# maxwerhahn/Multi-pass-GAN

Measured on AMD Instinct MI355X. Metric: volumes/sec (4x two-pass generator inference, 64^3->256^3 density-only), higher is better.
Workload: dtype f16+2xbf6->f32

## Files before the change

multi-pass-gan_amd/csrc/mpgan_conv_f6.hip:

```cpp
#include "mpgan_conv.h"

using namespace mpg::conv;

namespace {

#ifndef MPG_AH
#define MPG_AH 2
#endif
#ifndef MPG_WD
#define MPG_WD 1
#endif
#ifndef MPG_DIAG6
#define MPG_DIAG6 0
#endif
#ifndef MPG_W0
#define MPG_W0 1
#endif
#ifndef MPG_IMG_LATE
#define MPG_IMG_LATE 0
#endif
#ifndef MPG_PIECES_AFTER
#define MPG_PIECES_AFTER 1
#endif
#ifndef MPG_ALT
#define MPG_ALT 0
#endif
#ifndef MPG_STAMPS
#define MPG_STAMPS 0
#endif
#if MPG_STAMPS
#define MPG_STAMP(v) asm volatile("s_memtime %0" : "=s"(v))
#else
#define MPG_STAMP(v)
#endif
constexpr int lo_step(int pt, int nt, int ptn) {
    const int s = nt - ptn + pt - 1;
    return s < 0 ? 0 : (s > nt - 1 ? nt - 1 : s);
}

typedef int v16i __attribute__((ext_vector_type(16)));
typedef int v8i __attribute__((ext_vector_type(8)));
typedef int v6i __attribute__((ext_vector_type(6)));
typedef _Float16 half32 __attribute__((ext_vector_type(32)));
typedef _Float16 half16 __attribute__((ext_vector_type(16)));

__device__ __forceinline__ v8i lds_read32(const char* p) {
    const v4i lo = *reinterpret_cast<const v4i*>(p);
    const v4i hi = *reinterpret_cast<const v4i*>(p + 1024);
    return __builtin_shufflevector(lo, hi, 0, 1, 2, 3, 4, 5, 6, 7);
}

template <int OFF, class T>
__device__ __forceinline__ void ds_read16(T& dst, unsigned addr) {
    static_assert(sizeof(T) == 16 && OFF >= 0 && OFF < 65536, "one ds_read_b128");
    asm volatile("ds_read_b128 %0, %1 offset:%2" : "=v"(dst) : "v"(addr), "n"(OFF));
}

constexpr int kx_cum(int h, int NT, int PT) { return h + PT * ((h + NT - 1) / NT); }
constexpr int kx_allowed(int g, int NT, int PT, int AH) {
    const int G16 = 4 * NT;
    const int hi = g + AH + 1 < G16 ? g + AH + 1 : G16;
    return kx_cum(hi, NT, PT) - kx_cum(g + 1, NT, PT);
}

__device__ __forceinline__ half32 cat32(const half8& a, const half8& b, const half8& c, const half8& d) {
    const half16 lo = __builtin_shufflevector(a, b, 0, 1, 2, 3, 4, 5, 6, 7, 8, 9, 10, 11, 12, 13, 14, 15);
    const half16 hi = __builtin_shufflevector(c, d, 0, 1, 2, 3, 4, 5, 6, 7, 8, 9, 10, 11, 12, 13, 14, 15);
    return __builtin_shufflevector(lo, hi, 0, 1, 2, 3, 4, 5, 6, 7, 8, 9, 10, 11, 12, 13, 14, 15, 16, 17, 18, 19, 20, 21, 22, 23,
                                   24, 25, 26, 27, 28, 29, 30, 31);
}

__device__ __forceinline__ int block_exp16(const half32& v) {
    const v16i r = __builtin_bit_cast(v16i, v);
    int a0, a1, a2, a3, a4, a5, a6, a7, b0, b1, b2, b3, b4, b5, b6, b7, m2, m1;
#define MPG_MAX3(d, x, y, z) asm("v_pk_maximum3_f16 %0, %1, %2, %3" : "=v"(d) : "v"(x), "v"(y), "v"(z))
#define MPG_MIN3(d, x, y, z) asm("v_pk_minimum3_f16 %0, %1, %2, %3" : "=v"(d) : "v"(x), "v"(y), "v"(z))
    MPG_MAX3(a0, r[0], r[1], r[2]); MPG_MAX3(a1, r[3], r[4], r[5]); MPG_MAX3(a2, r[6], r[7], r[8]); MPG_MAX3(a3, r[9], r[10], r[11]);
    MPG_MAX3(a4, r[12], r[13], r[14]); MPG_MAX3(a5, a0, a1, r[15]); MPG_MAX3(a6, a2, a3, a4); MPG_MAX3(a7, a5, a6, a6);
    MPG_MIN3(b0, r[0], r[1], r[2]); MPG_MIN3(b1, r[3], r[4], r[5]); MPG_MIN3(b2, r[6], r[7], r[8]); MPG_MIN3(b3, r[9], r[10], r[11]);
    MPG_MIN3(b4, r[12], r[13], r[14]); MPG_MIN3(b5, b0, b1, r[15]); MPG_MIN3(b6, b2, b3, b4); MPG_MIN3(b7, b5, b6, b6);
#undef MPG_MAX3
#undef MPG_MIN3
    asm("v_pk_max_f16 %0, %1, %2 neg_lo:[0,1] neg_hi:[0,1]" : "=v"(m2) : "v"(a7), "v"(b7));
    asm("v_pk_max_f16 %0, %1, %1 op_sel:[0,1] op_sel_hi:[1,0]" : "=v"(m1) : "v"(m2));
    return (m1 >> 10) & 31;
}

#ifndef MPG_CVT_DIVIDES
#define MPG_CVT_DIVIDES 1
#endif
__device__ __forceinline__ float pow2_from_byte(int e8m0) {
#if MPG_CVT_DIVIDES
    return __builtin_bit_cast(float, e8m0 << 23);
#else
    return __builtin_bit_cast(float, (254 - e8m0) << 23);
#endif
}
__device__ __forceinline__ v8i widen6(const v6i& v) {
    return __builtin_shufflevector(v, v, 0, 1, 2, 3, 4, 5, -1, -1);
}
__device__ __forceinline__ v8i bf6_of(const half32& v, int e8m0) {
    return widen6(__builtin_amdgcn_cvt_scalef32_pk32_bf6_f16(v, pow2_from_byte(e8m0)));
}
constexpr int BF6 = 3;

template <int NT>
__global__ __launch_bounds__(Pipe6<NT>::WAVES * 64, Pipe6<NT>::OCC) void conv_mfma_f6_kernel(const ConvArgs a_unused) {
    extern __shared__ __attribute__((aligned(16))) char smem[];
    const KArgs ap = (KArgs)__builtin_amdgcn_kernarg_segment_ptr();
    const auto& a = *ap;
    using P = Pipe6<NT>;
    constexpr int WAVES = P::WAVES, PT = P::PT, TH = P::TH, WF16 = P::WF16, WF6 = P::WF6, WSTAGE = P::WSTAGE;
    constexpr int NI = P::NI, R = P::R, D = P::D, THREADS = WAVES * 64;
    constexpr bool FLAT = NT == 1;

    int* tap16 = reinterpret_cast<int*>(smem);
    char* img_lds = smem + a.tap_bytes;
    char* w_lds = img_lds + 2 * a.img_bytes;

    const int tid = threadIdx.x;
    const int lane = tid & 63;
    const int wave = tid >> 6;
    const int wave_u = __builtin_amdgcn_readfirstlane(wave);
    const int r = lane & 31;
    const int hh = lane >> 5;

    int bid = blockIdx.x;
    const int nblk = gridDim.x;
    if ((nblk & 7) == 0) bid = (bid & 7) * (nblk >> 3) + (bid >> 3);
    const int tx = bid % a.tiles_x;
    const int t2 = bid / a.tiles_x;
    const int ty = t2 % a.tiles_y;
    const int n = t2 / a.tiles_y;
    const int y0 = ty * TH, x0 = tx * TW;

    f32x16 acc[PT][NT];
#pragma unroll
    for (int pt = 0; pt < PT; ++pt)
#pragma unroll
        for (int nt = 0; nt < NT; ++nt)
#pragma unroll
            for (int i = 0; i < 16; ++i) acc[pt][nt][i] = 0.f;

    const EpiPre pre = epilogue_prefetch(ap, tid);
    const int seg_flip = (NT == 1 && a.nseg > 1) ? ((int)(blockIdx.x >> 8) & 1) : 0;
    for (int s0 = 0; s0 < ((a.dbg & 1) ? 0 : a.nseg); ++s0) {
        const int s = seg_flip ? a.nseg - 1 - s0 : s0;
        const auto& sg = ap->seg[s];
        if (NT <= 2 && sg.direct) {
            const unsigned plane_bytes = (unsigned)(sg.hs * sg.ws) * 16u;
            const unsigned gstride = 2u * plane_bytes;
            const char* xb = sg.x + ((size_t)n * sg.cg_total + sg.g_off) * gstride;
            unsigned pixo[PT];
#pragma unroll
            for (int pt = 0; pt < PT; ++pt) {
                int yy = y0 + PT * wave + pt, xx = x0 + r;
                yy = (yy < a.h ? yy : a.h - 1) >> sg.upy;
                xx = (xx < a.w ? xx : a.w - 1) >> sg.up;
                pixo[pt] = (unsigned)(yy * sg.ws + xx) * 16u;
            }
            const int glast = sg.cg_seg - 1;
            auto dma_stage_d = [&](int stage) {
                const int sidx = stage < sg.sc ? stage : sg.sc - 1;
                const char* src = sg.w + (size_t)sidx * WSTAGE + tid * 16;
                char* dst = w_lds + (stage % R) * WSTAGE + wave_u * 1024;
#pragma unroll
                for (int i = 0; i < NI; ++i) dma16(src + i * (THREADS * 16), dst + i * (THREADS * 16));
            };
#pragma unroll
            for (int d = 0; d < D; ++d) dma_stage_d(d);
            for (int st = 0; st < sg.sc; ++st) {
                wait_dma_and_barrier<(D - 1) * NI>();
                dma_stage_d(st + D);
                const char* wb = w_lds + (st % R) * WSTAGE;
                const char* xs = xb + (size_t)st * 8 * gstride;
                const int grem = glast - st * 8;
                if constexpr (FLAT) {
                    const unsigned a_base = lds_off(wb) + (unsigned)lane * 16u;
                    const char* xs_hi = xs;
                    const char* xs_lo = xs + plane_bytes;
                    asm volatile("" : "+s"(xs_hi), "+s"(xs_lo));
                    static_for<0, PT>([&](auto qc) {
                        constexpr int q = decltype(qc)::value;
                        half8 b_hi[4], b_lo[4], aq[2];
                        v4i wl[2], wh[2];
#pragma unroll
                        for (int j = 0; j < 4; ++j) {
                            int g = 2 * j + hh;
                            g = g < grem ? g : grem;
                            const unsigned vo = pixo[q] + g * gstride;
                            typedef const __attribute__((address_space(1))) half8* gmem;
                            b_hi[j] = __builtin_nontemporal_load((gmem)(xs_hi + vo));
                            b_lo[j] = __builtin_nontemporal_load((gmem)(xs_lo + vo));
                        }
                        ds_read16<0>(aq[0], a_base);
                        ds_read16<1024>(aq[1], a_base);
                        static_for<0, 4>([&](auto jc) {
                            constexpr int j = decltype(jc)::value;
                            lgkm_wait<(j < 3 ? 1 : 2)>();
                            tie(aq[j & 1]);
                            acc[q][0] = __builtin_amdgcn_mfma_f32_32x32x16_f16(aq[j & 1], b_hi[j], acc[q][0], 0, 0, 0);
                            if constexpr (j < 2) {
                                ds_read16<(j + 2) * 1024>(aq[j & 1], a_base);
                            } else if constexpr (j == 2) {
                                ds_read16<WF16 + WF6>(wl[0], a_base);
                                ds_read16<WF16 + WF6 + 1024>(wl[1], a_base);
                            } else {
                                ds_read16<WF16>(wh[0], a_base);
                                ds_read16<WF16 + 1024>(wh[1], a_base);
                            }
                        });
                        const half32 bh = cat32(b_hi[0], b_hi[1], b_hi[2], b_hi[3]);
                        const int e = block_exp16(bh);
                        const v8i hi6 = bf6_of(bh, e + 109);
                        const v8i lo6 = bf6_of(cat32(b_lo[0], b_lo[1], b_lo[2], b_lo[3]), e + 97);
                        const int sb = (e + 109) | (e + 97) << 8;
                        lgkm_wait<2>();
                        tie(wl[0]);
                        tie(wl[1]);
                        const v8i w_lo = __builtin_shufflevector(wl[0], wl[1], 0, 1, 2, 3, 4, 5, 6, 7);
                        acc[q][0] = __builtin_amdgcn_mfma_scale_f32_32x32x64_f8f6f4(w_lo, hi6, acc[q][0], BF6, BF6, 1, w_lo[6], 0, sb);
                        lgkm_wait<0>();
                        tie(wh[0]);
                        tie(wh[1]);
                        const v8i w_hi = __builtin_shufflevector(wh[0], wh[1], 0, 1, 2, 3, 4, 5, 6, 7);
                        acc[q][0] = __builtin_amdgcn_mfma_scale_f32_32x32x64_f8f6f4(w_hi, lo6, acc[q][0], BF6, BF6, 0, w_hi[6], 1, sb);
                    });
                    continue;
                }
                constexpr int PH = 2;
                static_for<0, PT / PH>([&](auto hc) {
                    constexpr int p0 = decltype(hc)::value * PH;
                    half8 b_hi[4][PH], b_lo[4][PH];
#pragma unroll
                    for (int j = 0; j < 4; ++j) {
                        int g = 2 * j + hh;
                        g = g < grem ? g : grem;
#pragma unroll
                        for (int q = 0; q < PH; ++q) {
                            b_hi[j][q] = __builtin_nontemporal_load(reinterpret_cast<const half8*>(xs + (pixo[p0 + q] + g * gstride)));
                            b_lo[j][q] = __builtin_nontemporal_load(reinterpret_cast<const half8*>(xs + (pixo[p0 + q] + g * gstride + plane_bytes)));
                        }
                    }
#pragma unroll
                    for (int j = 0; j < 4; ++j) {
#pragma unroll
                        for (int nt = 0; nt < NT; ++nt) {
                            const half8 a_hi = *reinterpret_cast<const half8*>(wb + ((j * NT + nt) * 64 + lane) * 16);
#pragma unroll
                            for (int q = 0; q < PH; ++q)
                                acc[p0 + q][nt] = __builtin_amdgcn_mfma_f32_32x32x16_f16(a_hi, b_hi[j][q], acc[p0 + q][nt], 0, 0, 0);
                        }
                    }
                    v8i hi6[PH], lo6[PH];
                    int sb[PH];
#pragma unroll
                    for (int q = 0; q < PH; ++q) {
                        const half32 bh = cat32(b_hi[0][q], b_hi[1][q], b_hi[2][q], b_hi[3][q]);
                        const half32 bl = cat32(b_lo[0][q], b_lo[1][q], b_lo[2][q], b_lo[3][q]);
                        const int e = block_exp16(bh);
                        hi6[q] = bf6_of(bh, e + 109);
                        lo6[q] = bf6_of(bl, e + 97);
                        sb[q] = (e + 109) | (e + 97) << 8;
                    }
#pragma unroll
                    for (int nt = 0; nt < NT; ++nt) {
                        const v8i w_hi = lds_read32(wb + WF16 + nt * 2048 + lane * 16);
                        const v8i w_lo = lds_read32(wb + WF16 + WF6 + nt * 2048 + lane * 16);
#pragma unroll
                        for (int q = 0; q < PH; ++q) {
                            acc[p0 + q][nt] = __builtin_amdgcn_mfma_scale_f32_32x32x64_f8f6f4(w_lo, hi6[q], acc[p0 + q][nt], BF6, BF6, 1, w_lo[6], 0, sb[q]);
                            acc[p0 + q][nt] = __builtin_amdgcn_mfma_scale_f32_32x32x64_f8f6f4(w_hi, lo6[q], acc[p0 + q][nt], BF6, BF6, 0, w_hi[6], 1, sb[q]);
                        }
                    }
                });
            }
            asm volatile("s_waitcnt vmcnt(0)" ::: "memory");
            __syncthreads();
            if constexpr (!FLAT) continue;
        }
        if constexpr (FLAT) {
            if (__builtin_amdgcn_readfirstlane(sg.direct)) continue;
        }
        const int T = sg.kh * sg.kw;
        const int G = sg.nchunks;
        const int NS = sg.sc;
        const int plane_b = sg.np * 16;
        const int ppg = sg.np >> 6;

        for (int q = tid; q < NS * 8; q += THREADS) {
            const int g = q / sg.tp;
            const int t = q - g * sg.tp;
            int off = ((g < G ? g : G - 1) & 1) * a.img_bytes;
            if (g < G && t < T) {
                const int dy = t / sg.kw;
                const int dx = t - dy * sg.kw;
                off += (dy * sg.iw + dx) * 16;
            }
            tap16[(q >> 3) * 8 + (q & 1) * 4 + ((q & 7) >> 1)] = off;
        }
        int pixb[PT];
#pragma unroll
        for (int pt = 0; pt < PT; ++pt) pixb[pt] = ((PT * wave + pt) * sg.iw + r) * 16;

        const size_t plane_px = (size_t)sg.hs * sg.ws;
        constexpr int MAXI = 4;
        static_assert(WAVES == 8, "MAXI");
        int img_src[MAXI];
#pragma unroll
        for (int i = 0; i < MAXI; ++i) {
            const int pc = WAVES * i + wave_u;
            const int pl = pc / ppg;
            const int p = (pc - pl * ppg) * 64 + lane;
            const int hy = p / sg.iw;
            const int hx = p - hy * sg.iw;
            const int yy = y0 - sg.pt + hy;
            const int xx = x0 - sg.pl + hx;
            const bool ok = pl < 2 && hy < sg.ih && yy >= 0 && yy < a.h && xx >= 0 && xx < a.w;
            img_src[i] = ok ? (int)(((size_t)pl * plane_px + (size_t)(yy >> sg.upy) * sg.ws + (xx >> sg.up)) * 16) : -1;
        }
        const size_t group_bytes = 2 * plane_px * 16;
        const char* const x_first = sg.x + ((size_t)n * sg.cg_total + sg.g_off) * group_bytes;
        auto img_piece = [&](int chunk, auto ic) {
            constexpr int i = decltype(ic)::value;
            if ((MPG_DIAG6 & 4) && chunk > 0) return;
            if (i < sg.ni_img) {
                const int off = img_src[i];
                const char* src = (off >= 0 && chunk < sg.cg_seg) ? x_first + (size_t)chunk * group_bytes + off : a.zeros;
                dma16_stream(src, img_lds + (chunk & 1) * a.img_bytes + (WAVES * i + wave_u) * 1024);
            }
        };
        auto w_piece = [&](int stage, auto ic) {
            constexpr int i = decltype(ic)::value;
            const int sidx = stage < NS ? stage : NS - 1;
            if ((MPG_DIAG6 & 8) && stage >= D) return;
            dma16(sg.w + (size_t)sidx * WSTAGE + tid * 16 + i * (THREADS * 16),
                  w_lds + (stage % R) * WSTAGE + wave_u * 1024 + i * (THREADS * 16));
        };
        static_for<0, MAXI>([&](auto ic) { img_piece(0, ic); });
#pragma unroll
        for (int d = 0; d < D; ++d) static_for<0, NI>([&](auto ic) { w_piece(d, ic); });
        int g_next = 1;

        half8 bh[PT][4];
        v4i o16n = {0, 0, 0, 0};
        const unsigned i_base = lds_off(img_lds);
#if MPG_STAMPS
        unsigned long long ts0 = 0, ts1 = 0, ts2 = 0, ts3 = 0, ts3_prev = 0;
        unsigned sum_head = 0, sum_f16 = 0, sum_f6 = 0, sum_bar = 0;
#endif

        auto run_stages = [&](auto oc) {
        constexpr bool CORR_FIRST = decltype(oc)::value != 0;
        int img_in_flight = 0;
        for (int st = 0; st < NS; ++st) {
            if constexpr (MPG_IMG_LATE) wait_dma_rt((D - 1) * NI, img_in_flight);
            else wait_dma_and_barrier<(D - 1) * NI>();
#if MPG_STAMPS
            if (st > 0) {
                sum_head += (unsigned)(ts1 - ts0);
                sum_f16 += (unsigned)(ts2 - ts1);
                sum_f6 += (unsigned)(ts3 - ts2);
                if (st > 1) sum_bar += (unsigned)(ts0 - ts3_prev);
                ts3_prev = ts3;
            }
            MPG_STAMP(ts0);
#endif
            if (st == 0) {
                ds_read16<0>(o16n, lds_off(tap16 + hh * 4));
                lgkm_wait<0>();
            }
            tie(o16n);
            const v4i o16 = o16n;
            const int to16[4] = {o16.x, o16.y, o16.z, o16.w};
            {
                const int sn = st + 1 < NS ? st + 1 : st;
                ds_read16<0>(o16n, lds_off(tap16 + (sn * 2 + hh) * 4));
            }
            const bool do_img = g_next < G && st * 8 >= (g_next - 1) * sg.tp;
            const int img_chunk = g_next;
            img_in_flight = (MPG_IMG_LATE && do_img && (g_next * sg.tp) / 8 >= st + 2) ? sg.ni_img : 0;
            if (do_img) ++g_next;
            const char* wb = w_lds + (st % R) * WSTAGE;
            const unsigned a_base = lds_off(wb) + (unsigned)lane * 16u;
            constexpr int AH = MPG_AH, G16 = 4 * NT;
            half8 aq[AH + 1];
            v8i hi6[PT], lo6[PT];
            int sb[PT], e16[PT];
            auto read_group = [&](auto gc) {
                constexpr int g = decltype(gc)::value, j = g / NT;
                if constexpr (g % NT == 0)
                    static_for<0, PT>([&](auto pc) {
                        constexpr int pt = decltype(pc)::value;
                        ds_read16<0>(bh[pt][j], i_base + (unsigned)(pixb[pt] + to16[j]));
                    });
                ds_read16<g * 1024>(aq[g % (AH + 1)], a_base);
            };
            auto make_hi6 = [&](auto pc) {
                constexpr int pt = decltype(pc)::value;
#if MPG_DIAG6 & 2
                const v4i q0 = __builtin_bit_cast(v4i, bh[pt][0]), q1 = __builtin_bit_cast(v4i, bh[pt][1]);
                hi6[pt] = __builtin_shufflevector(q0, q1, 0, 1, 2, 3, 4, 5, 6, 7);
                e16[pt] = 15;
                sb[pt] = 0x7f7f7f7f;
#else
                const half32 b32 = cat32(bh[pt][0], bh[pt][1], bh[pt][2], bh[pt][3]);
                e16[pt] = block_exp16(b32);
                hi6[pt] = bf6_of(b32, e16[pt] + 109);
                sb[pt] = (e16[pt] + 109) | (e16[pt] + 97) << 8;
#endif
            };
            constexpr int HALF = G16 / 2;
            constexpr int IPG = (MAXI + HALF - 1) / HALF;
            constexpr int WPG = (NI + HALF - 1) / HALF;
            constexpr int KS6 = 2 * NT;
            constexpr int WD = MPG_WD < KS6 - 1 ? MPG_WD : KS6 - 1;
            v4i wq[WD + 1][2];
            auto read_w6 = [&](auto kc) {
                constexpr int k = decltype(kc)::value;
                constexpr int off = WF16 + (k < NT ? WF6 + k * 2048 : (k - NT) * 2048);
                ds_read16<off>(wq[k % (WD + 1)][0], a_base);
                ds_read16<off + 1024>(wq[k % (WD + 1)][1], a_base);
            };
            auto fp16_phase = [&](auto mk) {
                constexpr bool MAKE_HI6 = decltype(mk)::value != 0;
                constexpr bool W0_AHEAD = MAKE_HI6 && MPG_W0;
                static_for<0, (AH < G16 ? AH : G16)>([&](auto gc) { read_group(gc); });
                static_for<0, G16>([&](auto gc) {
                    constexpr int g = decltype(gc)::value, j = g / NT, nt = g % NT;
                    auto pieces = [&]() {
                        if constexpr (g < HALF) {
                            if (do_img)
                                static_for<0, IPG>([&](auto kc) {
                                    constexpr int i = g * IPG + decltype(kc)::value;
                                    if constexpr (i < MAXI) img_piece(img_chunk, std::integral_constant<int, i>{});
                                });
                        } else {
                            static_for<0, WPG>([&](auto kc) {
                                constexpr int i = (g - HALF) * WPG + decltype(kc)::value;
                                if constexpr (i < NI) w_piece(st + D, std::integral_constant<int, i>{});
                            });
                        }
                    };
                    if constexpr (!MPG_PIECES_AFTER) pieces();
                    if constexpr (g + AH < G16) read_group(std::integral_constant<int, g + AH>{});
                    if constexpr (W0_AHEAD && g == G16 - 1) read_w6(std::integral_constant<int, 0>{});
                    lgkm_wait<kx_allowed(g, NT, PT, AH) + (W0_AHEAD && g == G16 - 1 ? 2 : 0)>();
                    if constexpr (g == 0 && MAKE_HI6) { MPG_STAMP(ts1); }
                    tie(aq[g % (AH + 1)]);
                    if constexpr (nt == 0)
                        static_for<0, PT>([&](auto pc) { tie(bh[decltype(pc)::value][j]); });
                    static_for<0, PT>([&](auto pc) {
                        constexpr int pt = decltype(pc)::value;
                        acc[pt][nt] = __builtin_amdgcn_mfma_f32_32x32x16_f16(aq[g % (AH + 1)], bh[pt][j], acc[pt][nt], 0, 0, 0);
                    });
                    if constexpr (MPG_PIECES_AFTER) pieces();
                    if constexpr (MAKE_HI6) {
                        if constexpr (g >= 3 * NT && g - 3 * NT < PT) make_hi6(std::integral_constant<int, g - 3 * NT>{});
                        if constexpr (g == G16 - 1 && NT < PT) static_for<NT, PT>([&](auto pc) { make_hi6(pc); });
                    }
                });
            };
            auto bf6_phase = [&](auto w0c) {
            constexpr bool W0_DONE = decltype(w0c)::value != 0;
#if !(MPG_DIAG6 & 1)
            constexpr int PB = PT;
            auto read_bl = [&](auto pc) {
                constexpr int pt = decltype(pc)::value;
                static_for<0, 4>([&](auto jc) {
                    constexpr int j = decltype(jc)::value;
                    ds_read16<0>(bh[pt][j], i_base + (unsigned)(plane_b + pixb[pt] + to16[j]));
                });
            };
            auto make_lo6 = [&](auto pc) {
                constexpr int pt = decltype(pc)::value;
                static_for<0, 4>([&](auto jc) { tie(bh[pt][decltype(jc)::value]); });
#if MPG_DIAG6 & 2
                const v4i q0 = __builtin_bit_cast(v4i, bh[pt][0]), q1 = __builtin_bit_cast(v4i, bh[pt][1]);
                lo6[pt] = __builtin_shufflevector(q0, q1, 0, 1, 2, 3, 4, 5, 6, 7);
#else
                lo6[pt] = bf6_of(cat32(bh[pt][0], bh[pt][1], bh[pt][2], bh[pt][3]), e16[pt] + 97);
#endif
            };
            if constexpr (!W0_DONE) read_w6(std::integral_constant<int, 0>{});
            static_for<0, PB>([&](auto pc) { read_bl(pc); });
            static_for<1, WD + 1>([&](auto kc) { read_w6(kc); });
            static_for<0, KS6>([&](auto kc) {
                constexpr int k = decltype(kc)::value;
                if constexpr (k >= 1 && k + WD < KS6) read_w6(std::integral_constant<int, k + WD>{});
                constexpr int ahead = (k + WD < KS6 ? k + WD : KS6 - 1) - k;
                lgkm_wait<(k == 0 ? 4 * PB : 0) + 2 * ahead>();
                tie(wq[k % (WD + 1)][0]);
                tie(wq[k % (WD + 1)][1]);
                const v8i w6 = __builtin_shufflevector(wq[k % (WD + 1)][0], wq[k % (WD + 1)][1], 0, 1, 2, 3, 4, 5, 6, 7);
                static_for<0, PT>([&](auto pc) {
                    constexpr int pt = decltype(pc)::value;
                    if constexpr (k < NT)
                        acc[pt][k] = __builtin_amdgcn_mfma_scale_f32_32x32x64_f8f6f4(w6, hi6[pt], acc[pt][k], BF6, BF6, 1, w6[6], 0, sb[pt]);
                    else
                        acc[pt][k - NT] = __builtin_amdgcn_mfma_scale_f32_32x32x64_f8f6f4(w6, lo6[pt], acc[pt][k - NT], BF6, BF6, 0, w6[6], 1, sb[pt]);
                });
                if constexpr (k < NT) {
                    if constexpr (k == 0 && lo_step(0, NT, PT) == 0) lgkm_wait<2 * ahead>();
                    static_for<0, PT>([&](auto pc) {
                        if constexpr (lo_step(decltype(pc)::value, NT, PT) == k) make_lo6(pc);
                    });
                }
            });
#else
            const v8i& h0 = hi6[0];
            const int &s0 = sb[0], &e0 = e16[0];
            asm volatile("" ::"v"(h0), "v"(s0), "v"(e0));
#endif
            };
            if constexpr (CORR_FIRST) {
                static_for<0, PT>([&](auto pc) {
                    constexpr int pt = decltype(pc)::value;
                    static_for<0, 4>([&](auto jc) {
                        constexpr int j = decltype(jc)::value;
                        ds_read16<0>(bh[pt][j], i_base + (unsigned)(pixb[pt] + to16[j]));
                    });
                });
                lgkm_wait<0>();
                static_for<0, PT>([&](auto pc) {
                    static_for<0, 4>([&](auto jc) { tie(bh[decltype(pc)::value][decltype(jc)::value]); });
                    make_hi6(pc);
                });
                MPG_STAMP(ts1);
                bf6_phase(std::integral_constant<int, 0>{});
                MPG_STAMP(ts2);
                fp16_phase(std::integral_constant<int, 0>{});
            } else {
                fp16_phase(std::integral_constant<int, 1>{});
                MPG_STAMP(ts2);
                bf6_phase(std::integral_constant<int, MPG_W0>{});
            }
            MPG_STAMP(ts3);
        }
        };
#if MPG_ALT
        if (WAVES == 8 && wave_u >= WAVES / 2) run_stages(std::integral_constant<int, 1>{});
        else
#endif
            run_stages(std::integral_constant<int, 0>{});
        asm volatile("s_waitcnt vmcnt(0) lgkmcnt(0)" ::: "memory");
        __syncthreads();
#if MPG_STAMPS
        if ((a.dbg & 8) && a.y != nullptr && s == 0 && lane == 0) {
            unsigned* o = reinterpret_cast<unsigned*>(a.y) + ((size_t)blockIdx.x * WAVES + wave) * 4;
            o[0] = sum_head; o[1] = sum_f16; o[2] = sum_f6; o[3] = sum_bar;
        }
#endif
    }
    conv_epilogue<NT, PT>(acc, ap, smem, n, y0, x0, wave, lane, pre);
}

}

hipError_t mpg::conv::launch_conv_f6(int nt, dim3 grid, size_t lds, hipStream_t st, const ConvArgs& a) {
    switch (nt) {
        case 1: return mpg::launch_dyn_lds<conv_mfma_f6_kernel<1>>(grid, dim3(Pipe6<1>::WAVES * 64), lds, st, a);
        case 2: return mpg::launch_dyn_lds<conv_mfma_f6_kernel<2>>(grid, dim3(Pipe6<2>::WAVES * 64), lds, st, a);
        case 3: return mpg::launch_dyn_lds<conv_mfma_f6_kernel<3>>(grid, dim3(Pipe6<3>::WAVES * 64), lds, st, a);
        default: return mpg::launch_dyn_lds<conv_mfma_f6_kernel<4>>(grid, dim3(Pipe6<4>::WAVES * 64), lds, st, a);
    }
}
```

multi-pass-gan_amd/csrc/mpgan_mfma_dev.h:

```cpp
#pragma once
#include <hip/hip_runtime.h>
#include <type_traits>

namespace mpg::dev {

typedef _Float16 half8 __attribute__((ext_vector_type(8)));
typedef float f32x16 __attribute__((ext_vector_type(16)));

typedef int v4i __attribute__((ext_vector_type(4)));

template <int N>
__device__ __forceinline__ void wait_dma_and_barrier() {
    asm volatile("s_waitcnt vmcnt(%0) lgkmcnt(0)\n\ts_barrier" ::"n"(N) : "memory");
}
__device__ __forceinline__ void wait_dma_rt(int base, int extra) {
    switch (base + extra) {
#define MPG_W(n) case n: wait_dma_and_barrier<n>(); break;
        MPG_W(0) MPG_W(1) MPG_W(2) MPG_W(3) MPG_W(4) MPG_W(5) MPG_W(6) MPG_W(7) MPG_W(8) MPG_W(9) MPG_W(10) MPG_W(11)
        MPG_W(12) MPG_W(13) MPG_W(14) MPG_W(15)
#undef MPG_W
        default: wait_dma_and_barrier<0>(); break;
    }
}

__device__ __forceinline__ void dma16(const char* src, char* lds_wave_base) {
    __builtin_amdgcn_global_load_lds((const __attribute__((address_space(1))) void*)src,
                                     (__attribute__((address_space(3))) void*)lds_wave_base, 16, 0, 0);
}

__device__ __forceinline__ void dma16_stream(const char* src, char* lds_wave_base) {
    __builtin_amdgcn_global_load_lds((const __attribute__((address_space(1))) void*)src,
                                     (__attribute__((address_space(3))) void*)lds_wave_base, 16, 0, 2);
}

template <int I, int N, class F>
__device__ __forceinline__ void static_for(F&& f) {
    if constexpr (I < N) {
        f(std::integral_constant<int, I>{});
        static_for<I + 1, N>(f);
    }
}
__device__ __forceinline__ unsigned lds_off(const void* p) {
    return (unsigned)(size_t)(const __attribute__((address_space(3))) char*)p;
}
template <int N>
__device__ __forceinline__ void lgkm_wait() {
    asm volatile("s_waitcnt lgkmcnt(%0)" ::"n"(N < 15 ? N : 15) : "memory");
}
template <class T>
__device__ __forceinline__ void tie(T& frag) {
    asm volatile("" : "+v"(frag));
}

}
```

Measured before the change: 15.61.

## Move stage barrier mid-iteration and prefetch next stage's head during bf6 phase

New measurement: 15.81, median of 6. 1.3% higher.

```diff
diff --git a/multi-pass-gan_amd/csrc/mpgan_conv_f6.hip b/multi-pass-gan_amd/csrc/mpgan_conv_f6.hip
--- a/multi-pass-gan_amd/csrc/mpgan_conv_f6.hip
+++ b/multi-pass-gan_amd/csrc/mpgan_conv_f6.hip
@@ -16,14 +16,8 @@
 #ifndef MPG_W0
 #define MPG_W0 1
 #endif
-#ifndef MPG_IMG_LATE
-#define MPG_IMG_LATE 0
-#endif
 #ifndef MPG_PIECES_AFTER
 #define MPG_PIECES_AFTER 1
-#endif
-#ifndef MPG_ALT
-#define MPG_ALT 0
 #endif
 #ifndef MPG_STAMPS
 #define MPG_STAMPS 0
@@ -122,8 +116,6 @@
     const int lane = tid & 63;
     const int wave = tid >> 6;
     const int wave_u = __builtin_amdgcn_readfirstlane(wave);
-    const int r = lane & 31;
-    const int hh = lane >> 5;
 
     int bid = blockIdx.x;
     const int nblk = gridDim.x;
@@ -147,6 +139,9 @@
     for (int s0 = 0; s0 < ((a.dbg & 1) ? 0 : a.nseg); ++s0) {
         const int s = seg_flip ? a.nseg - 1 - s0 : s0;
         const auto& sg = ap->seg[s];
+        int tid_seg = threadIdx.x;
+        asm volatile("" : "+v"(tid_seg));
+        const int tid = tid_seg, lane = tid & 63, wave = tid >> 6, r = lane & 31, hh = lane >> 5;
         if (NT <= 2 && sg.direct) {
             const unsigned plane_bytes = (unsigned)(sg.hs * sg.ws) * 16u;
             const unsigned gstride = 2u * plane_bytes;
@@ -345,30 +340,57 @@
         half8 bh[PT][4];
         v4i o16n = {0, 0, 0, 0};
         const unsigned i_base = lds_off(img_lds);
+        constexpr int AH = MPG_AH, G16 = 4 * NT;
+        half8 aq[AH + 1];
+        constexpr int NAH = AH < G16 ? AH : G16;
+        constexpr int NPG = NT == 1 ? 0 : NAH;
+        constexpr int NPRE = kx_cum(NPG, NT, PT);
+        auto prefetch_head = [&](int stage, const v4i& o) {
+            const unsigned ab = lds_off(w_lds + (stage % R) * WSTAGE) + (unsigned)lane * 16u;
+            const int t[4] = {o.x, o.y, o.z, o.w};
+            static_for<0, NPG>([&](auto gc) {
+                constexpr int g = decltype(gc)::value, j = g / NT;
+                if constexpr (g % NT == 0)
+                    static_for<0, PT>([&](auto pc) {
+                        constexpr int pt = decltype(pc)::value;
+                        ds_read16<0>(bh[pt][j], i_base + (unsigned)(pixb[pt] + t[j]));
+                    });
+                ds_read16<g * 1024>(aq[g % (AH + 1)], ab);
+            });
+        };
 #if MPG_STAMPS
         unsigned long long ts0 = 0, ts1 = 0, ts2 = 0, ts3 = 0, ts3_prev = 0;
         unsigned sum_head = 0, sum_f16 = 0, sum_f6 = 0, sum_bar = 0;
 #endif
 
-        auto run_stages = [&](auto oc) {
-        constexpr bool CORR_FIRST = decltype(oc)::value != 0;
-        int img_in_flight = 0;
+        auto run_stages = [&](auto mc) {
+        constexpr bool MID = decltype(mc)::value != 0;
+        if constexpr (MID) {
+            wait_dma_and_barrier<(D - 1) * NI>();
+            ds_read16<0>(o16n, lds_off(tap16 + hh * 4));
+            lgkm_wait<0>();
+            tie(o16n);
+            prefetch_head(0, o16n);
+        }
         for (int st = 0; st < NS; ++st) {
-            if constexpr (MPG_IMG_LATE) wait_dma_rt((D - 1) * NI, img_in_flight);
-            else wait_dma_and_barrier<(D - 1) * NI>();
+            if constexpr (!MID) wait_dma_and_barrier<(D - 1) * NI>();
 #if MPG_STAMPS
-            if (st > 0) {
-                sum_head += (unsigned)(ts1 - ts0);
-                sum_f16 += (unsigned)(ts2 - ts1);
-                sum_f6 += (unsigned)(ts3 - ts2);
-                if (st > 1) sum_bar += (unsigned)(ts0 - ts3_prev);
-                ts3_prev = ts3;
-            }
-            MPG_STAMP(ts0);
-#endif
-            if (st == 0) {
-                ds_read16<0>(o16n, lds_off(tap16 + hh * 4));
-                lgkm_wait<0>();
+            if constexpr (!MID) {
+                if (st > 0) {
+                    sum_head += (unsigned)(ts1 - ts0);
+                    sum_f16 += (unsigned)(ts2 - ts1);
+                    sum_f6 += (unsigned)(ts3 - ts2);
+                    if (st > 1) sum_bar += (unsigned)(ts0 - ts3_prev);
+                    ts3_prev = ts3;
+                }
+                MPG_STAMP(ts0);
+            }
+#endif
+            if constexpr (!MID) {
+                if (st == 0) {
+                    ds_read16<0>(o16n, lds_off(tap16 + hh * 4));
+                    lgkm_wait<0>();
+                }
             }
             tie(o16n);
             const v4i o16 = o16n;
@@ -377,14 +399,13 @@
                 const int sn = st + 1 < NS ? st + 1 : st;
                 ds_read16<0>(o16n, lds_off(tap16 + (sn * 2 + hh) * 4));
             }
-            const bool do_img = g_next < G && st * 8 >= (g_next - 1) * sg.tp;
+            const int st_free = MID ? st - 1 : st;
+            const bool do_img = st_free >= 0 && g_next < G && st_free * 8 >= (g_next - 1) * sg.tp;
             const int img_chunk = g_next;
-            img_in_flight = (MPG_IMG_LATE && do_img && (g_next * sg.tp) / 8 >= st + 2) ? sg.ni_img : 0;
+            const int img_late = (MID && !(MPG_DIAG6 & 4) && do_img && (g_next * sg.tp) / 8 > st + 1) ? sg.ni_img : 0;
             if (do_img) ++g_next;
             const char* wb = w_lds + (st % R) * WSTAGE;
             const unsigned a_base = lds_off(wb) + (unsigned)lane * 16u;
-            constexpr int AH = MPG_AH, G16 = 4 * NT;
-            half8 aq[AH + 1];
             v8i hi6[PT], lo6[PT];
             int sb[PT], e16[PT];
             auto read_group = [&](auto gc) {
@@ -415,6 +436,7 @@
             constexpr int WPG = (NI + HALF - 1) / HALF;
             constexpr int KS6 = 2 * NT;
             constexpr int WD = MPG_WD < KS6 - 1 ? MPG_WD : KS6 - 1;
+            constexpr int WPC = (NI + NT - 1) / NT;
             v4i wq[WD + 1][2];
             auto read_w6 = [&](auto kc) {
                 constexpr int k = decltype(kc)::value;
@@ -422,10 +444,9 @@
                 ds_read16<off>(wq[k % (WD + 1)][0], a_base);
                 ds_read16<off + 1024>(wq[k % (WD + 1)][1], a_base);
             };
-            auto fp16_phase = [&](auto mk) {
-                constexpr bool MAKE_HI6 = decltype(mk)::value != 0;
-                constexpr bool W0_AHEAD = MAKE_HI6 && MPG_W0;
-                static_for<0, (AH < G16 ? AH : G16)>([&](auto gc) { read_group(gc); });
+            auto fp16_phase = [&]() {
+                constexpr bool W0_AHEAD = MPG_W0 != 0;
+                static_for<(MID ? NPG : 0), NAH>([&](auto gc) { read_group(gc); });
                 static_for<0, G16>([&](auto gc) {
                     constexpr int g = decltype(gc)::value, j = g / NT, nt = g % NT;
                     auto pieces = [&]() {
@@ -435,7 +456,7 @@
                                     constexpr int i = g * IPG + decltype(kc)::value;
                                     if constexpr (i < MAXI) img_piece(img_chunk, std::integral_constant<int, i>{});
                                 });
-                        } else {
+                        } else if constexpr (!MID) {
                             static_for<0, WPG>([&](auto kc) {
                                 constexpr int i = (g - HALF) * WPG + decltype(kc)::value;
                                 if constexpr (i < NI) w_piece(st + D, std::integral_constant<int, i>{});
@@ -445,8 +466,8 @@
                     if constexpr (!MPG_PIECES_AFTER) pieces();
                     if constexpr (g + AH < G16) read_group(std::integral_constant<int, g + AH>{});
                     if constexpr (W0_AHEAD && g == G16 - 1) read_w6(std::integral_constant<int, 0>{});
-                    lgkm_wait<kx_allowed(g, NT, PT, AH) + (W0_AHEAD && g == G16 - 1 ? 2 : 0)>();
-                    if constexpr (g == 0 && MAKE_HI6) { MPG_STAMP(ts1); }
+                    lgkm_wait<kx_allowed(g, NT, PT, AH) + (W0_AHEAD && g == G16 - 1 ? 2 : 0) + (MID && g < NPG ? 1 : 0)>();
+                    if constexpr (g == 0 && !MID) { MPG_STAMP(ts1); }
                     tie(aq[g % (AH + 1)]);
                     if constexpr (nt == 0)
                         static_for<0, PT>([&](auto pc) { tie(bh[decltype(pc)::value][j]); });
@@ -455,10 +476,8 @@
                         acc[pt][nt] = __builtin_amdgcn_mfma_f32_32x32x16_f16(aq[g % (AH + 1)], bh[pt][j], acc[pt][nt], 0, 0, 0);
                     });
                     if constexpr (MPG_PIECES_AFTER) pieces();
-                    if constexpr (MAKE_HI6) {
-                        if constexpr (g >= 3 * NT && g - 3 * NT < PT) make_hi6(std::integral_constant<int, g - 3 * NT>{});
-                        if constexpr (g == G16 - 1 && NT < PT) static_for<NT, PT>([&](auto pc) { make_hi6(pc); });
-                    }
+                    if constexpr (g >= 3 * NT && g - 3 * NT < PT) make_hi6(std::integral_constant<int, g - 3 * NT>{});
+                    if constexpr (g == G16 - 1 && NT < PT) static_for<NT, PT>([&](auto pc) { make_hi6(pc); });
                 });
             };
             auto bf6_phase = [&](auto w0c) {
@@ -489,7 +508,13 @@
                 constexpr int k = decltype(kc)::value;
                 if constexpr (k >= 1 && k + WD < KS6) read_w6(std::integral_constant<int, k + WD>{});
                 constexpr int ahead = (k + WD < KS6 ? k + WD : KS6 - 1) - k;
-                lgkm_wait<(k == 0 ? 4 * PB : 0) + 2 * ahead>();
+                constexpr int pre = (MID && k == KS6 - 1) ? NPRE : 0;
+                if constexpr (pre != 0) {
+                    tie(o16n);
+                    prefetch_head(st + 1, o16n);
+                }
+                lgkm_wait<(k == 0 ? 4 * PB : 0) + 2 * ahead + pre>();
+                if constexpr (k == 0 && MID) { MPG_STAMP(ts1); }
                 tie(wq[k % (WD + 1)][0]);
                 tie(wq[k % (WD + 1)][1]);
                 const v8i w6 = __builtin_shufflevector(wq[k % (WD + 1)][0], wq[k % (WD + 1)][1], 0, 1, 2, 3, 4, 5, 6, 7);
@@ -505,44 +530,47 @@
                     static_for<0, PT>([&](auto pc) {
                         if constexpr (lo_step(decltype(pc)::value, NT, PT) == k) make_lo6(pc);
                     });
+                } else if constexpr (MID) {
+                    static_for<0, WPC>([&](auto ic) {
+                        constexpr int i = (k - NT) * WPC + decltype(ic)::value;
+                        if constexpr (i < NI) w_piece(st + D, std::integral_constant<int, i>{});
+                    });
                 }
             });
 #else
+            if constexpr (MID) static_for<0, NI>([&](auto ic) { w_piece(st + D, ic); });
             const v8i& h0 = hi6[0];
             const int &s0 = sb[0], &e0 = e16[0];
             asm volatile("" ::"v"(h0), "v"(s0), "v"(e0));
 #endif
             };
-            if constexpr (CORR_FIRST) {
-                static_for<0, PT>([&](auto pc) {
-                    constexpr int pt = decltype(pc)::value;
-                    static_for<0, 4>([&](auto jc) {
-                        constexpr int j = decltype(jc)::value;
-                        ds_read16<0>(bh[pt][j], i_base + (unsigned)(pixb[pt] + to16[j]));
-                    });
-                });
-                lgkm_wait<0>();
-                static_for<0, PT>([&](auto pc) {
-                    static_for<0, 4>([&](auto jc) { tie(bh[decltype(pc)::value][decltype(jc)::value]); });
-                    make_hi6(pc);
-                });
-                MPG_STAMP(ts1);
-                bf6_phase(std::integral_constant<int, 0>{});
-                MPG_STAMP(ts2);
-                fp16_phase(std::integral_constant<int, 0>{});
-            } else {
-                fp16_phase(std::integral_constant<int, 1>{});
-                MPG_STAMP(ts2);
-                bf6_phase(std::integral_constant<int, MPG_W0>{});
-            }
+            fp16_phase();
+            MPG_STAMP(ts2);
+            if constexpr (MID) {
+                wait_dma_late_and_barrier(img_late);
+#if MPG_STAMPS
+                if (st > 0) {
+                    sum_head += (unsigned)(ts1 - ts0);
+                    sum_f6 += (unsigned)(ts3 - ts1);
+                    sum_f16 += (unsigned)(ts2 - ts3);
+                    if (st > 1) sum_bar += (unsigned)(ts0 - ts3_prev);
+                    ts3_prev = ts2;
+                }
+                MPG_STAMP(ts0);
+#endif
+            }
+            bf6_phase(std::integral_constant<int, MPG_W0>{});
             MPG_STAMP(ts3);
         }
         };
-#if MPG_ALT
-        if (WAVES == 8 && wave_u >= WAVES / 2) run_stages(std::integral_constant<int, 1>{});
-        else
-#endif
+        if constexpr (NT == 1) {
             run_stages(std::integral_constant<int, 0>{});
+        } else {
+            int mid = __builtin_amdgcn_readfirstlane(sg.pref);
+            if (mid) run_stages(std::integral_constant<int, 1>{});
+            asm volatile("" : "+s"(mid));
+            if (!mid) run_stages(std::integral_constant<int, 0>{});
+        }
         asm volatile("s_waitcnt vmcnt(0) lgkmcnt(0)" ::: "memory");
         __syncthreads();
 #if MPG_STAMPS
diff --git a/multi-pass-gan_amd/csrc/mpgan_mfma_dev.h b/multi-pass-gan_amd/csrc/mpgan_mfma_dev.h
--- a/multi-pass-gan_amd/csrc/mpgan_mfma_dev.h
+++ b/multi-pass-gan_amd/csrc/mpgan_mfma_dev.h
@@ -13,14 +13,33 @@
 __device__ __forceinline__ void wait_dma_and_barrier() {
     asm volatile("s_waitcnt vmcnt(%0) lgkmcnt(0)\n\ts_barrier" ::"n"(N) : "memory");
 }
-__device__ __forceinline__ void wait_dma_rt(int base, int extra) {
-    switch (base + extra) {
-#define MPG_W(n) case n: wait_dma_and_barrier<n>(); break;
-        MPG_W(0) MPG_W(1) MPG_W(2) MPG_W(3) MPG_W(4) MPG_W(5) MPG_W(6) MPG_W(7) MPG_W(8) MPG_W(9) MPG_W(10) MPG_W(11)
-        MPG_W(12) MPG_W(13) MPG_W(14) MPG_W(15)
-#undef MPG_W
-        default: wait_dma_and_barrier<0>(); break;
-    }
+__device__ __forceinline__ void wait_dma_late_and_barrier(int late) {
+    asm volatile(
+        "s_cmp_lt_u32 %0, 1\n\t"
+        "s_cbranch_scc1 .Lmpg_w0_%=\n\t"
+        "s_cmp_lt_u32 %0, 2\n\t"
+        "s_cbranch_scc1 .Lmpg_w1_%=\n\t"
+        "s_cmp_lt_u32 %0, 3\n\t"
+        "s_cbranch_scc1 .Lmpg_w2_%=\n\t"
+        "s_cmp_lt_u32 %0, 4\n\t"
+        "s_cbranch_scc1 .Lmpg_w3_%=\n\t"
+        "s_waitcnt vmcnt(4)\n\t"
+        "s_branch .Lmpg_wb_%=\n"
+        ".Lmpg_w3_%=:\n\t"
+        "s_waitcnt vmcnt(3)\n\t"
+        "s_branch .Lmpg_wb_%=\n"
+        ".Lmpg_w2_%=:\n\t"
+        "s_waitcnt vmcnt(2)\n\t"
+        "s_branch .Lmpg_wb_%=\n"
+        ".Lmpg_w1_%=:\n\t"
+        "s_waitcnt vmcnt(1)\n\t"
+        "s_branch .Lmpg_wb_%=\n"
+        ".Lmpg_w0_%=:\n\t"
+        "s_waitcnt vmcnt(0)\n"
+        ".Lmpg_wb_%=:\n\t"
+        "s_waitcnt lgkmcnt(0)\n\t"
+        "s_barrier" ::"s"(late)
+        : "memory", "scc");
 }
 
 __device__ __forceinline__ void dma16(const char* src, char* lds_wave_base) {
```
